# waiwnf/pilotguru

Measured on AMD Instinct MI355X. Metric: frames/sec ORB extract+match, 1080p @ 2000 kp/frame, higher is better.
Workload: dtype u8

## Files before the change

include/pgorb.h:

```cpp
#ifndef PGORB_H
#define PGORB_H
#include <stdint.h>
#ifdef __cplusplus
extern "C" {
#endif

#define PGORB_MAX_LEVELS 16

enum {
    PGORB_OK = 0,
    PGORB_E_ARG = -1,
    PGORB_E_TOOSMALL = -2,
    PGORB_E_CAP = -3,
    PGORB_E_NODEVICE = -4,
    PGORB_E_HIP = -5,
    PGORB_E_LIMIT = -6,
    PGORB_E_OVERFLOW = -7
};

typedef struct pgorb_ctx pgorb_ctx;

typedef struct pgorb_params {
    int32_t nfeatures;
    float   scale_factor;
// ... 421 lines not shown
#define PGORB_OPTION_UNKNOWN (-2147483647 - 1)
int  pgorb_set_option(pgorb_ctx* ctx, const char* key, int value);
int  pgorb_get_option(const pgorb_ctx* ctx, const char* key);
int  pgorb_matcher_is_popcount(const pgorb_ctx* ctx, int cap_per_frame);

int  pgorb_profile_host(pgorb_ctx* ctx, double* us , int reset);

int  pgorb_debug_level_size(const pgorb_ctx* ctx, int level, int* w, int* h);
int  pgorb_debug_level_image(pgorb_ctx* ctx, int frame, int level, uint8_t* out );
int  pgorb_debug_level_candidates(pgorb_ctx* ctx, int frame, int level,
                                  int32_t* x, int32_t* y, int32_t* response, int cap);
int  pgorb_debug_level_keypoints(pgorb_ctx* ctx, int frame, int level);
int  pgorb_debug_sincos_checksum(uint32_t first_bits, uint32_t count, int nblocks, unsigned long long* out);

enum { PGORB_ARENA_STAGE_A = 0, PGORB_ARENA_PINNED = 1, PGORB_ARENA_SCRATCH = 2, PGORB_ARENA_STAGE_OUT = 3, PGORB_ARENA_XDESC = 4,
       PGORB_ARENA_OUT_BLOCK = 5, PGORB_ARENA_VOCAB = 6, PGORB_ARENA_PLAN_PYR = 7, PGORB_ARENA_PLAN_TABLES = 8 };
int  pgorb_debug_arena(const pgorb_ctx* ctx, int which, const void** ptr, int64_t* bytes);
int  pgorb_debug_host_graph(const pgorb_ctx* ctx, int* last_call, int* plan_epoch);

#ifdef __cplusplus
}
#endif
#endif
```

pilotguru_amd/csrc/extract.hip:

```cpp
#include "pgorb_ctx.h"

#include <chrono>

namespace {

std::vector<hipEvent_t*> pipe_pyr_events(pgorb_ctx* c)
{
    std::vector<hipEvent_t*> v{&c->evFork, &c->evPyrDone, &c->evFastDone};
    for (hipEvent_t& e : c->evLevel) v.push_back(&e);
    return v;
}
std::vector<hipEvent_t*> pipe_lev_events(pgorb_ctx* c)
{
    std::vector<hipEvent_t*> v{&c->evDescDone};
    for (hipEvent_t& e : c->evGrpFast) v.push_back(&e);
    for (hipEvent_t& e : c->evGrpQt) v.push_back(&e);
    return v;
}
int make_side_streams(pgorb_ctx* c, hipStream_t* a, bool aHigh, hipStream_t* b, const std::vector<hipEvent_t*>& events)
{
    int lo = 0, hi = 0;
    PG_HIP(c, hipDeviceGetStreamPriorityRange(&lo, &hi));
    PG_HIP(c, hipStreamCreateWithPriority(a, hipStreamNonBlocking, aHigh ? hi : lo));
    PG_HIP(c, hipStreamCreateWithPriority(b, hipStreamNonBlocking, lo));
// ... 378 lines not shown

int pgorb_debug_level_keypoints(pgorb_ctx* c, int frame, int level)
{
    if (!tap_ok(c, level) || frame < 0 || frame >= c->lastFrames) return PGORB_E_ARG;
    PG_HIP(c, hipSetDevice(c->prm.device));
    PG_HIP(c, hipDeviceSynchronize());
    int32_t cnt = 0;
    PG_HIP(c, hipMemcpy(&cnt, c->plan.kpCount + frame * PG_MAXL + level, 4, hipMemcpyDeviceToHost));
    return cnt;
}

int pgorb_debug_arena(const pgorb_ctx* c, int which, const void** ptr, int64_t* bytes)
{
    if (!c || !ptr || !bytes) return PGORB_E_ARG;
    if (which == PGORB_ARENA_PINNED) { *ptr = c->pinned; *bytes = (int64_t)c->pinnedBytes; return 0; }
    const Arena* all[] = {&c->stageA, nullptr, &c->stageSfi, &c->stageOut, &c->xdesc, &c->outBlk, &c->vocab, &c->pyr, &c->tables};
    if (which < 0 || which >= (int)(sizeof(all) / sizeof(all[0]))) return PGORB_E_ARG;
    *ptr = all[which]->p; *bytes = (int64_t)all[which]->bytes;
    return 0;
}

int pgorb_debug_host_graph(const pgorb_ctx* c, int* last_call, int* plan_epoch)
{
    if (!c || !last_call || !plan_epoch) return PGORB_E_ARG;
    *last_call = c->hg.last; *plan_epoch = c->planEpoch;
    return 0;
}

}
```

pilotguru_amd/csrc/pgorb_internal.h:

```cpp
#pragma once
#include <hip/hip_runtime.h>
#include <stdint.h>
#include <string.h>
#include "../../include/pgorb.h"

#define PG_EDGE 16
#define PG_MAXL PGORB_MAX_LEVELS

struct PgQuadTab {
    int32_t  base_dw;
    uint32_t offs;
    int16_t  a0[4], a1[4];
};

struct PgQuadTab2 {
    int32_t  xb;
    uint32_t sel[4];
    uint32_t coef[4];
};

struct PgRowGrp {
    int32_t  sFirst;
    uint32_t yrel4;
    int16_t  ybeta[8];
// ... 79 lines not shown
    uint2*    qtLeaf;
    int32_t   qtSplit;
    int32_t   qtThreads;
    int32_t   qtWide;
    int32_t*  status;
};

#define QT_PYR_CAP 4096
__host__ __device__ __forceinline__ int qt_pyr_off(int nIni, int d) { return nIni * (((1 << (2 * d)) - 1) / 3); }
__host__ __device__ __forceinline__ int qt_pyr_depth(int nIni)
{
    int D = 5;
    while (D > 0 && qt_pyr_off(nIni, D + 1) > QT_PYR_CAP) D--;
    return D;
}
#if defined(__HIP_DEVICE_COMPILE__)
#define PG_FDIV_RN(a, b) __fdiv_rn(a, b)
#define PG_FMUL_RN(a, b) __fmul_rn(a, b)
#else
#define PG_FDIV_RN(a, b) ((a) / (b))
#define PG_FMUL_RN(a, b) ((a) * (b))
#endif
__host__ __device__ inline uint2 qt_tab_entry(bool isY, int c, float hX, int nIni, int regionH, int D, int wCell, int hCell, int nCols)
{
    const uint32_t mW = ((1u << 20) + wCell - 1) / wCell, mH = ((1u << 20) + hCell - 1) / hCell;
    int part, a0, a1;
    if (isY) { part = 0; a0 = 0; a1 = regionH; }
    else {
        int r = nIni >= 1 ? (int)PG_FDIV_RN((float)c, hX) : 0;
        const int top = (nIni > 1 ? nIni : 1) - 1;
// ... 154 lines not shown
```

pilotguru_amd/csrc/plan.hip:

```cpp
#include "pgorb_ctx.h"

static inline int cvRound(double v) { return (int)lrint(v); }
static inline int cvFloor(double v) { int i = (int)v; return i - (v < i); }

int level_geometry(const pgorb_ctx* c, int w, int h, LevelGeom* g)
{
    for (int l = 0; l < c->prm.nlevels; l++) {
        const float scale = c->mvInvScaleFactor[l];
        g[l].w = cvRound((double)((float)w * scale)); g[l].h = cvRound((double)((float)h * scale));
        const float width = (float)(g[l].w - 2 * PG_EDGE), height = (float)(g[l].h - 2 * PG_EDGE);
        const int nCols = (int)(width / 30.f), nRows = (int)(height / 30.f);
        if (nCols < 1 || nRows < 1) return PGORB_E_TOOSMALL;
        g[l].nCols = nCols; g[l].nRows = nRows;
        g[l].wCell = (int)ceilf(width / nCols);
        g[l].hCell = (int)ceilf(height / nRows);
        const int rw = g[l].w - 2 * PG_EDGE, rh = g[l].h - 2 * PG_EDGE;
        g[l].nIni = (int)roundf((float)rw / rh);
        if (g[l].nIni < 1) g[l].nIni = 0;
        g[l].hX = g[l].nIni ? (float)rw / g[l].nIni : 0.f;
    }
    return 0;
}

namespace {
// ... 208 lines not shown
        A.pyrOff[l] = A.pyrFrame;
        A.pyrFrame += (size_t)V.fstride;
        V.nCols = g[l].nCols; V.nRows = g[l].nRows; V.wCell = g[l].wCell; V.hCell = g[l].hCell;
        V.cellBase = A.cells; A.cells += V.nCols * V.nRows;
        V.quota = c->mnFeaturesPerLevel[l];
        V.nIni = g[l].nIni; V.hX = g[l].hX;
        V.selCap = std::max(V.quota + 2, 4 * V.nIni);
        V.nodeCap = (int)align_up(V.selCap + 8, 4);
        V.candCap = ((V.w - 2 * PG_EDGE) / 2 + V.nCols + 1) * ((V.h - 2 * PG_EDGE) / 2 + V.nRows + 1);
        V.candOff = (int64_t)A.candFrame; A.candFrame += align_up(V.candCap, 64);
        V.cellCap = ((V.wCell + 1) / 2) * ((V.hCell + 1) / 2);
        V.cellCandOff = (int64_t)A.cellCandFrame;
        A.cellCandFrame += align_up((size_t)V.cellCap * V.nCols * V.nRows, 64);
        V.selOff = (int64_t)A.selFrame; A.selFrame += V.selCap;
        V.nodeOff = -1;
        const size_t qtAux = std::max((size_t)3072, (size_t)g[0].nCols * g[0].nRows + 1);
        const size_t qtTab = (size_t)2 * ((g[0].w - 2 * PG_EDGE) + (g[0].h - 2 * PG_EDGE));
        if (std::max((size_t)V.nodeCap * 28, qtTab) * sizeof(int) + qtAux * sizeof(int) + 17 * 1024 > 160 * 1024) {
            V.nodeOff = (int64_t)A.nodeFrame;
            A.nodeFrame += align_up((size_t)V.nodeCap * 30, 64);
        }
        V.scale = c->mvScaleFactor[l];
        V.patchSize = (float)(int)(31 * c->mvScaleFactor[l]);
        A.selTotal += V.selCap;
        if ((size_t)(V.nCols * V.nRows + 1) * sizeof(int) > 140 * 1024)
            return fail(c, PGORB_E_LIMIT, "too many cells on one level for the quadtree kernel's LDS budget");
        if (V.w > 4095 + 2 * PG_EDGE || V.h > 4095 + 2 * PG_EDGE)
            return fail(c, PGORB_E_LIMIT, "level larger than 4095 px is not supported");
        if (V.selCap > 65535)
            return fail(c, PGORB_E_LIMIT, "more than 65533 keypoints on one pyramid level are not supported");
    }
    A.selFrame = align_up(A.selFrame, 16);
    P.totalCells = A.cells; P.selTotal = A.selTotal;
    P.cellCandFrame = (int64_t)A.cellCandFrame;
    P.candFrame = (int64_t)A.candFrame; P.selFrame = (int64_t)A.selFrame; P.nodeFrame = (int64_t)A.nodeFrame;
// ... 187 lines not shown
```

pilotguru_amd/csrc/quadtree.hip:

```cpp
#include "pgorb_internal.h"

#define QT_TMAX 1024
#define QT_T ((int)blockDim.x)
#define QT_SH (__builtin_ctz(blockDim.x))
#define QT_W (QT_T >> 6)
#define QT_POS_MASK 0x0FFFFFFFu

#ifndef QT_HU
#define QT_HU 4
#endif
#define QT_SETTLE4(a, b, c, d) asm volatile("" : "+v"(a), "+v"(b), "+v"(c), "+v"(d))

__device__ __forceinline__ int qt_wave_incl_scan(int x)
{
    int v = x;
    v += __builtin_amdgcn_update_dpp(0, v, 0x111, 0xf, 0xf, true);
    v += __builtin_amdgcn_update_dpp(0, v, 0x112, 0xf, 0xf, true);
    v += __builtin_amdgcn_update_dpp(0, v, 0x114, 0xf, 0xf, true);
    v += __builtin_amdgcn_update_dpp(0, v, 0x118, 0xf, 0xf, true);
    v += __builtin_amdgcn_update_dpp(0, v, 0x142, 0xa, 0xf, false);
    v += __builtin_amdgcn_update_dpp(0, v, 0x143, 0xc, 0xf, false);
    return v;
}

__device__ int qt_scan_excl(int* a, int n, int* sh)
{
    const int tid = threadIdx.x, lane = tid & 63, wv = tid >> 6;
    const int per = (n + QT_T - 1) >> QT_SH;
    const int b = tid * per, e = min(b + per, n);
    int sum = 0;
    for (int i = b; i < e; i++) sum += a[i];
    const int incl = qt_wave_incl_scan(sum);
    if (lane == 63) sh[wv] = incl;
    __syncthreads();
    if (wv == 0) {
        const int v = (lane < QT_W) ? sh[lane] : 0;
        const int w = qt_wave_incl_scan(v);
        if (lane < QT_W) sh[lane] = w - v;
        if (lane == QT_W - 1) sh[QT_W] = w;
    }
    __syncthreads();
    int run = sh[wv] + incl - sum;
    for (int i = b; i < e; i++) { const int v = a[i]; a[i] = run; run += v; }
    const int total = sh[QT_W];
    __syncthreads();
    return total;
}

__device__ __forceinline__ void qt_scan3_threads(int& a, int& b, int& c, int* tot, int* sh)
{
    const int tid = threadIdx.x, lane = tid & 63, wv = tid >> 6;
    const int ia = qt_wave_incl_scan(a), ib = qt_wave_incl_scan(b), ic = qt_wave_incl_scan(c);
    if (lane == 63) { sh[wv] = ia; sh[QT_W + wv] = ib; sh[2 * QT_W + wv] = ic; }
    __syncthreads();
    int pa = 0, pb = 0, pc = 0, ta = 0, tb = 0, tc = 0;
    for (int w = 0; w < QT_W; w++) {
        const int va = sh[w], vb = sh[QT_W + w], vc = sh[2 * QT_W + w];
        if (w < wv) { pa += va; pb += vb; pc += vc; }
// ... 4 lines not shown
    __syncthreads();
}

__device__ __forceinline__ void qt_wave_count(int* ctr, int target, bool active)
{
    const unsigned long long todo = __ballot(active);
    if (todo == 0) return;
    const int leader = __ffsll((long long)todo) - 1;
    const int t = __builtin_amdgcn_readlane(target, leader);
    if (__ballot(active && target != t) == 0) {
        if ((int)(threadIdx.x & 63) == leader) atomicAdd(&ctr[t], __popcll(todo));
    } else if (active) {
        atomicAdd(&ctr[target], 1);
    }
}

__device__ __forceinline__ int qt_quadrant(const int4 b, uint32_t cv)
{
    const int midX = b.x + ((b.z - b.x + 1) >> 1);
    const int midY = b.y + ((b.w - b.y + 1) >> 1);
    const int x = cv & 0xFFF, y = (cv >> 12) & 0xFFF;
    return (x < midX) ? ((y < midY) ? 0 : 2) : ((y < midY) ? 1 : 3);
}


__device__ __forceinline__ int qt_leaf(uint32_t cv, float hX, int nIni, int regionH, int D)
{
    const int x = cv & 0xFFF, y = (cv >> 12) & 0xFFF;
    int r = (int)__fdiv_rn((float)x, hX);
    r = min(max(r, 0), nIni - 1);
// ... 9 lines not shown
    return idx;
}

__device__ __forceinline__ int qt_walk(const int* map, int leaf, int nIni, int D)
{
    for (int d = 0; d <= D; d++) {
        const int m = map[qt_pyr_off(nIni, d) + (leaf >> (2 * (D - d)))];
        if (m >= 0) return m;
    }
    return 0;
}

__device__ __forceinline__ int qt_build_keys(const int32_t* __restrict__ cc, const uint32_t* __restrict__ slots, int ncells, int cellCap,
                                             int* cellOff, int* sh, uint2* keys, float hX, int nIni, int regionH, int D)
{
    const int tid = threadIdx.x;
    for (int i = tid; i < ncells; i += QT_T) cellOff[i] = min(cc[i], cellCap);
    __syncthreads();
    const int ncand = qt_scan_excl(cellOff, ncells, sh);
    if (tid == 0) cellOff[ncells] = ncand;
    __syncthreads();
    int steps = 0;
    while ((1 << steps) < ncells) steps++;
    for (int b0 = 0; b0 < ncand; b0 += QT_HU * QT_T) {
        int lo[QT_HU], hi[QT_HU];
#pragma unroll
        for (int u = 0; u < QT_HU; u++) { lo[u] = 0; hi[u] = ncells - 1; }
        for (int st = 0; st < steps; st++) {
#pragma unroll
            for (int u = 0; u < QT_HU; u++) {
                const int mid = (lo[u] + hi[u] + 1) >> 1;
                const bool le = cellOff[mid] <= b0 + u * QT_T + tid;
                lo[u] = le ? mid : lo[u];
                hi[u] = le ? hi[u] : mid - 1;
            }
        }
        uint32_t v[QT_HU];
#pragma unroll
// ... 2 lines not shown
            v[u] = (i < ncand) ? slots[(int64_t)lo[u] * cellCap + (i - cellOff[lo[u]])] : 0u;
        }
        QT_SETTLE4(v[0], v[1], v[2], v[3]);
        if (QT_HU == 8) QT_SETTLE4(v[4 % QT_HU], v[5 % QT_HU], v[6 % QT_HU], v[7 % QT_HU]);
#pragma unroll
        for (int u = 0; u < QT_HU; u++) {
            const int i = b0 + u * QT_T + tid;
            if (i < ncand) keys[i] = make_uint2(v[u], (uint32_t)qt_leaf(v[u], hX, nIni, regionH, D));
        }
    }
    __syncthreads();
    return ncand;
}

template <bool BIG, int WIDE>
__global__ __launch_bounds__((WIDE == 1 || WIDE == 3) ? 512 : QT_TMAX, WIDE == 3 ? 6 : (WIDE ? 4 : 8)) void k_quadtree(const PgPlan P, int level0, int leafOffInts, int split)
{
    __shared__ int sh[3 * (QT_TMAX / 64) + 8];
    __shared__ int pyr[QT_PYR_CAP];
    extern __shared__ __attribute__((aligned(16))) int qt_lds[];
    const int tid = threadIdx.x;
    const int l = level0 + blockIdx.y, frame = blockIdx.x;
    const PgLevel& L = P.lvl[l];
    int* kpc = &P.kpCount[frame * PG_MAXL + l];
    uint2* keys = reinterpret_cast<uint2*>(P.cand) + ((int64_t)frame * P.candFrame + L.candOff);
    if (BIG != (L.nodeOff >= 0)) return;
    const int NC = L.nodeCap;
    int* nodeBase = BIG ? P.nodeScratch + (int64_t)frame * P.nodeFrame + L.nodeOff : qt_lds;
    int4* bndA = reinterpret_cast<int4*>(nodeBase);
    int4* bndB = bndA + NC;
    int* cntA = reinterpret_cast<int*>(bndB + NC);
    int* cntB = cntA + NC;
    int* pidA = cntB + NC;
    int* pidB = pidA + NC;
    int* cnt4 = pidB + NC;
    int* cnt4n = cnt4 + 4 * NC;
    int* newpos4 = cnt4n + 4 * NC;
    int* tailpos = newpos4 + 4 * NC;
    int* rnk = tailpos + NC;
    int* ord = rnk + NC;
    int* cinc = ord + NC;
    int* tmp = newpos4;
    int* ecnt = newpos4 + NC;
    unsigned long long* best = reinterpret_cast<unsigned long long*>(newpos4);
    uint32_t* leafBest = reinterpret_cast<uint32_t*>(qt_lds + leafOffInts);
    int* cellOff = qt_lds + leafOffInts;

    const int N = L.quota;
    const int regionH = L.h - 2 * PG_EDGE;
    const int nIni = L.nIni;
    const float hX = L.hX;
    const int D = qt_pyr_depth(nIni);
    const int pyrTotal = qt_pyr_off(nIni, D + 1);

    const int wCell = L.wCell, hCell = L.hCell, nCols = L.nCols;
    const uint32_t mW = ((1u << 20) + wCell - 1) / wCell, mH = ((1u << 20) + hCell - 1) / hCell;
    auto order_rank = [&](uint32_t cv) {
        const uint32_t x = (cv & 0xFFF) - 3, y = ((cv >> 12) & 0xFFF) - 3;
        const uint32_t cj = (x * mW) >> 20, ci = (y * mH) >> 20;
        return ((ci * nCols + cj) * hCell + (y - ci * hCell)) * wCell + (x - cj * wCell);
    };
// ... 10 lines not shown
        for (int i = tid; i < pyrTotal; i += QT_T) pyr[i] = 0;
        if (!split) for (int i = tid; i < nleaf; i += QT_T) leafBest[i] = 0u;
        if (tid == 0) sh[QT_W + 2] = 0;
        int mine = 0;
        const int lane = tid & 63;
        if (split) {
            __syncthreads();
            int* hDs = pyr + qt_pyr_off(nIni, D);
            uint2* gl = P.qtLeaf + ((int64_t)frame * P.nlevels + l) * PG_QT_LEAF_CAP;
            for (int i = tid; i < nleaf; i += QT_T) {
                const uint2 e = gl[i];
                hDs[i] = (int)e.x; leafBest[i] = e.y; mine += (int)e.x;
            }
        } else {
        const int regionW = L.w - 2 * PG_EDGE;
        uint2* xTab = reinterpret_cast<uint2*>(qt_lds);
        uint2* yTab = xTab + regionW;
        for (int i = tid; i < regionW + regionH; i += QT_T) {
            const bool isY = i >= regionW;
            const int c = isY ? i - regionW : i;
            (isY ? yTab : xTab)[c] = qt_tab_entry(isY, c, hX, nIni, regionH, D, wCell, hCell, nCols);
        }
        __syncthreads();
        int* hD = pyr + qt_pyr_off(nIni, D);
        const int wv = __builtin_amdgcn_readfirstlane(tid >> 6);
        const int cellCap = L.cellCap;
        struct __attribute__((packed, aligned(4))) U4 { uint32_t e[4]; };
        if (ncells < QT_T) {
            const int sub = lane >> 4, sl = lane & 15;
            const int cpw = (((ncells + QT_W - 1) >> (QT_SH - 6)) + 31) & ~31;
            const int cBeg = wv * cpw, cEnd = min(ncells, cBeg + cpw);
// ... 90 lines not shown
        for (int d = D - 1; d >= 0; d--) {
            const int* src = pyr + qt_pyr_off(nIni, d + 1);
            int* dst = pyr + qt_pyr_off(nIni, d);
            const int cnt = nIni << (2 * d);
            for (int j = tid; j < cnt; j += QT_T) dst[j] = src[4 * j] + src[4 * j + 1] + src[4 * j + 2] + src[4 * j + 3];
            __syncthreads();
        }
    }

    int size;
    {
        if (tid == 0) {
            int pos = 0;
            for (int i = 0; i < nIni; i++) {
                if (pyr[i] > 0) {
                    bndA[pos] = make_int4((int)__fmul_rn(hX, (float)i), 0,
                                          (int)__fmul_rn(hX, (float)(i + 1)), regionH);
                    cntA[pos] = pyr[i];
                    pidA[pos] = i;
                    pos++;
                }
            }
            sh[QT_W + 1] = pos;
        }
        __syncthreads();
        size = sh[QT_W + 1];
        if (D >= 1)
            for (int i = tid; i < 4 * size; i += QT_T) cnt4[i] = pyr[nIni + 4 * pidA[i >> 2] + (i & 3)];
        __syncthreads();
    }

    int sorted_mode = 0, gen = 1;
    bool last = false, pyrMode = true;
    while (!last) {
        if (pyrMode && gen > D) {
            if (!keysBuilt) {
                qt_build_keys(P.cellCount + (int64_t)frame * P.totalCells + L.cellBase, P.cellCand + (int64_t)frame * P.cellCandFrame + L.cellCandOff,
                              L.nCols * L.nRows, L.cellCap, cellOff, sh, keys, hX, nIni, regionH, D);
                keysBuilt = true;
            }
            for (int i = tid; i < pyrTotal; i += QT_T) pyr[i] = -1;
            for (int i = tid; i < 4 * size; i += QT_T) cnt4[i] = 0;
            __syncthreads();
            for (int p = tid; p < size; p += QT_T) {
                const int pid = pidA[p];
                pyr[qt_pyr_off(nIni, pid >> 28) + (pid & QT_POS_MASK)] = p;
            }
            __syncthreads();
            for (int i0 = 0; i0 < ncand; i0 += QT_T) {
                const int i = i0 + tid;
                bool act = i < ncand;
                int tgt = 0;
                if (act) {
                    const uint2 k = keys[i];
                    const int pos = qt_walk(pyr, (int)k.y, nIni, D);
                    uint32_t rec = (uint32_t)pos;
                    act = cntA[pos] > 1;
                    if (act) {
                        const int q = qt_quadrant(bndA[pos], k.x);
                        tgt = pos * 4 + q;
                        rec |= (uint32_t)q << 28;
                    }
                    keys[i].y = rec;
                }
                qt_wave_count(cnt4, tgt, act);
            }
            __syncthreads();
            pyrMode = false;
        }
        const int n = size, prevSize = size;
        const bool fill = pyrMode && gen + 1 <= D;
        const int fillOff = qt_pyr_off(nIni, min(gen + 1, D));
        int jstar = 0;
        if (!sorted_mode) {
// ... 3 lines not shown
            for (int p = pb; p < pe; p++)
                if (cntA[p] > 1) {
                    const int c0 = cnt4[4 * p], c1 = cnt4[4 * p + 1], c2 = cnt4[4 * p + 2], c3 = cnt4[4 * p + 3];
                    se++; sc += (c0 > 0) + (c1 > 0) + (c2 > 0) + (c3 > 0); sx += (c0 > 1) + (c1 > 1) + (c2 > 1) + (c3 > 1);
                }
            int tot[3];
            qt_scan3_threads(se, sc, sx, tot, sh);
            const int m = tot[0], Ctot = tot[1], nToExpand = tot[2];
            size = Ctot + (n - m);
            if (size > NC) { if (tid == 0) atomicExch(P.status, PGORB_E_OVERFLOW); size = min(size, NC); last = true; }
            if (size >= N || size == prevSize) last = true;
            else if (size + 3 * nToExpand > N) sorted_mode = 1;
            int re = se, ce = sc;
            for (int p = pb; p < pe; p++) {
                if (cntA[p] > 1) {
                    const int4 b = bndA[p];
                    const int midX = b.x + ((b.z - b.x + 1) >> 1);
                    const int midY = b.y + ((b.w - b.y + 1) >> 1);
                    const int cq[4] = {cnt4[4 * p], cnt4[4 * p + 1], cnt4[4 * p + 2], cnt4[4 * p + 3]};
                    const int c = (cq[0] > 0) + (cq[1] > 0) + (cq[2] > 0) + (cq[3] > 0);
                    const int cidx = (int)(((uint32_t)pidA[p] & (QT_POS_MASK >> 2)) * 4u);
                    int pos = Ctot - (ce + c);
                    if (pos >= 0 && pos + c <= NC) {
#pragma unroll
                        for (int q = 3; q >= 0; q--) {
                            if (cq[q] <= 0) continue;
                            bndB[pos] = make_int4((q & 1) ? midX : b.x, (q & 2) ? midY : b.y,
                                                  (q & 1) ? b.z : midX, (q & 2) ? b.w : midY);
                            cntB[pos] = cq[q];
                            pidB[pos] = (int)(((uint32_t)gen << 28) | (uint32_t)(cidx + q));
                            if (fill && cq[q] > 1) {
                                const int* h = pyr + fillOff + (cidx + q) * 4;
                                cnt4n[4 * pos] = h[0]; cnt4n[4 * pos + 1] = h[1]; cnt4n[4 * pos + 2] = h[2]; cnt4n[4 * pos + 3] = h[3];
                            }
                            newpos4[4 * p + q] = pos++;
                        }
                    }
                    rnk[p] = 0; re++; ce += c;
                } else {
                    const int pos = min(Ctot + (p - re), NC - 1);
                    bndB[pos] = bndA[p]; cntB[pos] = cntA[p]; pidB[pos] = pidA[p];
                    tailpos[p] = pos; rnk[p] = -1;
                }
            }
        } else {
            for (int p = tid; p < n; p += QT_T) rnk[p] = (cntA[p] > 1) ? 1 : 0;
            __syncthreads();
            const int m = qt_scan_excl(rnk, n, sh);
            if (BIG) {
                for (int p = tid; p < n; p += QT_T) {
                    if (cntA[p] > 1) { tmp[rnk[p]] = p; ecnt[rnk[p]] = cntA[p]; }
                    else rnk[p] = -1;
                }
                __syncthreads();
                for (int i = tid; i < m; i += QT_T) {
                    const int ci = ecnt[i];
                    int rank = 0;
                    for (int j = 0; j < m; j++) {
                        const int cj = ecnt[j];
                        rank += (cj > ci) || (cj == ci && j < i);
                    }
                    ord[rank] = tmp[i];
                    rnk[tmp[i]] = rank;
                }
                __syncthreads();
            } else {
                for (int p = tid; p < n; p += QT_T) {
                    if (cntA[p] > 1) { tmp[rnk[p]] = p; ecnt[rnk[p]] = (int)(((uint32_t)min(cntA[p], 0x1FFFFF) << 11) | (uint32_t)(2047 - rnk[p])); }
                    else rnk[p] = -1;
                }
                __syncthreads();
                const int m4 = m & ~3;
                for (int i = tid; i < m; i += QT_T) {
                    const uint32_t ki = (uint32_t)ecnt[i];
                    int rank = 0;
                    for (int j = 0; j < m4; j += 4) {
                        const uint4 k4 = *reinterpret_cast<const uint4*>(ecnt + j);
                        rank += (k4.x > ki) + (k4.y > ki) + (k4.z > ki) + (k4.w > ki);
                    }
                    for (int j = m4; j < m; j++) rank += (uint32_t)ecnt[j] > ki;
                    ord[rank] = tmp[i];
                    rnk[tmp[i]] = rank;
                }
                __syncthreads();
            }
            for (int r = tid; r < m; r += QT_T) {
                const int p = ord[r];
                cinc[r] = (cnt4[4 * p] > 0) + (cnt4[4 * p + 1] > 0) + (cnt4[4 * p + 2] > 0) + (cnt4[4 * p + 3] > 0);
            }
            __syncthreads();
            qt_scan_excl(cinc, m, sh);
            for (int r = tid; r < m; r += QT_T) {
                const int p = ord[r];
                cinc[r] += (cnt4[4 * p] > 0) + (cnt4[4 * p + 1] > 0) + (cnt4[4 * p + 2] > 0) + (cnt4[4 * p + 3] > 0);
            }
            if (tid == 0) sh[QT_W + 1] = m - 1;
            __syncthreads();
            for (int r = tid; r < m; r += QT_T) {
                const bool now = n + cinc[r] - (r + 1) >= N;
                const bool before = (r > 0) && (n + cinc[r - 1] - r >= N);
                if (now && !before) sh[QT_W + 1] = r;
            }
            __syncthreads();
            jstar = sh[QT_W + 1];
            const int Ctot = (m > 0) ? cinc[jstar] : 0;
            for (int p = tid; p < n; p += QT_T) tailpos[p] = (rnk[p] >= 0 && rnk[p] <= jstar) ? 0 : 1;
            __syncthreads();
            const int U = qt_scan_excl(tailpos, n, sh);
            for (int p = tid; p < n; p += QT_T) {
                const int r = rnk[p];
                if (r >= 0 && r <= jstar) {
                    const int4 b = bndA[p];
                    const int midX = b.x + ((b.z - b.x + 1) >> 1);
                    const int midY = b.y + ((b.w - b.y + 1) >> 1);
                    const int cq[4] = {cnt4[4 * p], cnt4[4 * p + 1], cnt4[4 * p + 2], cnt4[4 * p + 3]};
                    const int cidx = (int)(((uint32_t)pidA[p] & (QT_POS_MASK >> 2)) * 4u);
                    int pos = Ctot - cinc[r];
#pragma unroll
                    for (int q = 3; q >= 0; q--) {
                        if (cq[q] <= 0) continue;
                        bndB[pos] = make_int4((q & 1) ? midX : b.x, (q & 2) ? midY : b.y,
                                              (q & 1) ? b.z : midX, (q & 2) ? b.w : midY);
                        cntB[pos] = cq[q];
                        pidB[pos] = (int)(((uint32_t)gen << 28) | (uint32_t)(cidx + q));
                        if (fill && cq[q] > 1) {
                            const int* h = pyr + fillOff + (cidx + q) * 4;
                            cnt4n[4 * pos] = h[0]; cnt4n[4 * pos + 1] = h[1]; cnt4n[4 * pos + 2] = h[2]; cnt4n[4 * pos + 3] = h[3];
                        }
                        newpos4[4 * p + q] = pos++;
                    }
                } else {
                    const int pos = Ctot + tailpos[p];
                    bndB[pos] = bndA[p]; cntB[pos] = cntA[p]; pidB[pos] = pidA[p];
                    tailpos[p] = pos;
                    if (fill && cntA[p] > 1) {
                        cnt4n[4 * pos] = cnt4[4 * p]; cnt4n[4 * pos + 1] = cnt4[4 * p + 1];
                        cnt4n[4 * pos + 2] = cnt4[4 * p + 2]; cnt4n[4 * pos + 3] = cnt4[4 * p + 3];
                    }
                }
            }
            size = Ctot + U;
            if (size > NC) { if (tid == 0) atomicExch(P.status, PGORB_E_OVERFLOW); size = NC; last = true; }
            if (size >= N || size == prevSize) last = true;
        }
        if (!pyrMode) {
            for (int i = tid; i < 4 * size; i += QT_T) cnt4n[i] = 0;
            __syncthreads();
            for (int b0 = 0; b0 < ncand; b0 += 4 * QT_T) {
                uint2 kk[4];
#pragma unroll
                for (int u = 0; u < 4; u++) { const int i = b0 + tid + u * QT_T; kk[u] = (i < ncand) ? keys[i] : make_uint2(0u, 0u); }
        QT_SETTLE4(kk[0].x, kk[1].x, kk[2].x, kk[3].x); QT_SETTLE4(kk[0].y, kk[1].y, kk[2].y, kk[3].y);
                int tgt[4];
                bool act[4];
#pragma unroll
                for (int u = 0; u < 4; u++) {
                    const int i = b0 + tid + u * QT_T;
                    act[u] = i < ncand;
                    tgt[u] = 0;
                    if (act[u]) {
                        const uint2 k = kk[u];
                        const int pos = k.y & QT_POS_MASK, q = k.y >> 28;
                        const int r = rnk[pos];
                        const int np = (r >= 0 && r <= jstar) ? newpos4[4 * pos + q] : tailpos[pos];
                        uint32_t rec = (uint32_t)np;
                        act[u] = !last && cntB[np] > 1;
                        if (act[u]) {
                            const int q2 = qt_quadrant(bndB[np], k.x);
                            tgt[u] = np * 4 + q2;
                            rec |= (uint32_t)q2 << 28;
                        }
                        if (last) atomicMax(&reinterpret_cast<unsigned long long*>(cnt4n)[np], bid(k.x));
                        else keys[i].y = rec;
                    }
                }
#pragma unroll
                for (int u = 0; u < 4; u++) qt_wave_count(cnt4n, tgt[u], act[u]);
            }
        }
        __syncthreads();
        { int4* t4 = bndA; bndA = bndB; bndB = t4; int* t1 = cntA; cntA = cntB; cntB = t1;
          t1 = cnt4; cnt4 = cnt4n; cnt4n = t1; t1 = pidA; pidA = pidB; pidB = t1; }
        gen++;
    }

    if (pyrMode) {
        for (int p = tid; p < size; p += QT_T) best[p] = 0ull;
        int* leafPos = pyr + qt_pyr_off(nIni, D);
        for (int i = tid; i < pyrTotal; i += QT_T) pyr[i] = -1;
        __syncthreads();
        for (int p = tid; p < size; p += QT_T) {
            const int pid = pidA[p];
            pyr[qt_pyr_off(nIni, pid >> 28) + (pid & QT_POS_MASK)] = p;
        }
        __syncthreads();
        const int nleaf = nIni << (2 * D);
// ... 152 lines not shown
    }
    __syncthreads();
    uint2* gl = P.qtLeaf + ((int64_t)frame * P.nlevels + l) * PG_QT_LEAF_CAP;
    const uint32_t cmask = (1u << D) - 1;
    for (int i = tid; i < nh; i += QTP_T) {
        const uint32_t rl = (uint32_t)i / (uint32_t)ncol, col = (uint32_t)i - rl * (uint32_t)ncol, row = (uint32_t)r0 + rl;
        const uint32_t leaf = ((col >> D) << (2 * D)) + qt_spread_bits(col & cmask) + 2u * qt_spread_bits(row);
        gl[leaf] = make_uint2((uint32_t)hC[i], hB[i]);
    }
}

void pg_launch_quadtree(const PgPlan& P, int nframes, hipStream_t s) { pg_launch_quadtree_levels(P, nframes, 0, P.nlevels, s); }

void pg_launch_quadtree_levels(const PgPlan& P, int nframes, int levelBeg, int levelEnd, hipStream_t s)
{
    int nodes[2] = {0, 0}, aux[2] = {0, 0};
    bool any[2] = {false, false};
    for (int l = levelBeg; l < levelEnd; l++) {
        const int big = P.lvl[l].nodeOff >= 0 ? 1 : 0;
        const int cells = P.lvl[l].nCols * P.lvl[l].nRows + 1;
        const int nIni = max(P.lvl[l].nIni, 1);
        const int leaves = nIni << (2 * qt_pyr_depth(nIni));
        any[big] = true;
        aux[big] = max(aux[big], max(cells, leaves));
        nodes[big] = max(nodes[big], 2 * ((P.lvl[l].w - 2 * PG_EDGE) + (P.lvl[l].h - 2 * PG_EDGE)));
        if (!big) nodes[0] = max(nodes[0], P.lvl[l].nodeCap * 28);
    }
    static size_t configuredDev[64] = {0};
    int dev = 0;
    (void)hipGetDevice(&dev);
    size_t& configured = configuredDev[dev & 63];
    const int cells0 = P.lvl[levelBeg].nCols * P.lvl[levelBeg].nRows;
    const bool split = P.qtSplit == 1 || (P.qtSplit == 2 && cells0 >= 1500 && nframes <= 16 + (cells0 - 2304) * 12 / 6912);
    if (split) {
        int groups = 0;
        size_t lds = 0;
        for (int l = levelBeg; l < levelEnd; l++) {
            const PgLevel& V = P.lvl[l];
            const int D = qt_pyr_depth(V.nIni), ncells = V.nCols * V.nRows;
            groups += qt_pass_groups(ncells, D);
            lds = std::max(lds, (size_t)((V.w - 2 * PG_EDGE) + (V.h - 2 * PG_EDGE)) * 8 + (size_t)qt_pass_rows_per_group(ncells, D) * (std::max(V.nIni, 0) << D) * 8 + 2 * 64 * 4);
        }
        static size_t passConfigured[64] = {0};
        int dev0 = 0;
        (void)hipGetDevice(&dev0);
        if (lds > 48 * 1024 && lds > passConfigured[dev0 & 63]) {
            (void)hipFuncSetAttribute(reinterpret_cast<const void*>(k_qt_leaves), hipFuncAttributeMaxDynamicSharedMemorySize, (int)lds);
            passConfigured[dev0 & 63] = lds;
        }
        if (groups > 0)
            hipLaunchKernelGGL(k_qt_leaves, dim3(groups, nframes), dim3(QTP_T), lds, s, P, levelBeg, levelEnd - levelBeg);
    }
    for (int big = 0; big < 2; big++) {
        if (!any[big]) continue;
        const size_t lds = (size_t)(nodes[big] + aux[big]) * sizeof(int);
        const size_t ldsAll = lds + sizeof(int) * (QT_PYR_CAP + 3 * (QT_TMAX / 64) + 8);
        int threads = QT_TMAX;
        if (ldsAll <= 80 * 1024 && (cells0 < 1024 || (int64_t)nframes * (levelEnd - levelBeg) > 256)) threads = 512;
        if (P.qtThreads == 256 || P.qtThreads == 512 || P.qtThreads == 1024) threads = P.qtThreads;
        dim3 grid(nframes, levelEnd - levelBeg), block(threads);
        const int64_t problems = (int64_t)nframes * (levelEnd - levelBeg);
        int wide = 0;
        if (P.qtWide && threads == 512 && ldsAll > 54 * 1024) wide = 1;
        if (P.qtWide && threads == 512 && ldsAll > 40 * 1024 && ldsAll <= 54 * 1024) wide = 3;
        if (P.qtWide && threads == QT_TMAX && (ldsAll > 80 * 1024 || problems <= 256)) wide = 2;
        if (lds > configured) {
#define PG_QT_ATTR(B, W) (void)hipFuncSetAttribute(reinterpret_cast<const void*>(k_quadtree<B, W>), hipFuncAttributeMaxDynamicSharedMemorySize, (int)lds)
            PG_QT_ATTR(true, 0); PG_QT_ATTR(true, 1); PG_QT_ATTR(true, 2); PG_QT_ATTR(true, 3); PG_QT_ATTR(false, 0); PG_QT_ATTR(false, 1); PG_QT_ATTR(false, 2); PG_QT_ATTR(false, 3);
#undef PG_QT_ATTR
            configured = lds;
        }
#define PG_QT_LAUNCH(B, W) hipLaunchKernelGGL((k_quadtree<B, W>), grid, block, lds, s, P, levelBeg, nodes[big], split ? 1 : 0)
        if (big) { if (wide == 1) PG_QT_LAUNCH(true, 1); else if (wide == 2) PG_QT_LAUNCH(true, 2); else if (wide == 3) PG_QT_LAUNCH(true, 3); else PG_QT_LAUNCH(true, 0); }
        else { if (wide == 1) PG_QT_LAUNCH(false, 1); else if (wide == 2) PG_QT_LAUNCH(false, 2); else if (wide == 3) PG_QT_LAUNCH(false, 3); else PG_QT_LAUNCH(false, 0); }
#undef PG_QT_LAUNCH
    }
}
```

pilotguru_amd/orb.py:

```python
import ctypes as C
import weakref

import numpy as np

from . import _lib

KEYPOINT_DTYPE = np.dtype([("x", "<f4"), ("y", "<f4"), ("size", "<f4"), ("angle", "<f4"),
                           ("response", "<f4"), ("octave", "<i4"), ("class_id", "<i4")])
assert KEYPOINT_DTYPE.itemsize == 28


def _p(a):
    return C.c_void_p(a.ctypes.data)


def _arr(x, dtype, n, name, width=None):
    a = np.ascontiguousarray(x, dtype)
    if a.shape != ((n,) if width is None else (n, width)):
        raise ValueError("%s: shape %s, expected %s" % (name, a.shape, (n,) if width is None else (n, width)))
    return a


def _frame(F, name):
    return (_arr(F.mvKeysUndistorted, KEYPOINT_DTYPE, F.N, name + " keypoints"),
# ... 217 lines not shown
        w, h = self.debug_level_size(level)
        out = np.zeros((h, w), np.uint8)
        self._check(self._L.pgorb_debug_level_image(self._h, frame, level, _p(out)))
        return out

    def debug_level_candidates(self, frame, level):
        w, h = self.debug_level_size(level)
        cap = w * h // 2 + 64
        x, y, r = (np.zeros(cap, np.int32) for _ in range(3))
        n = self._check(self._L.pgorb_debug_level_candidates(self._h, frame, level, _p(x), _p(y), _p(r), cap))
        return x[:n].copy(), y[:n].copy(), r[:n].copy()

    def debug_level_keypoints(self, frame, level):
        return self._check(self._L.pgorb_debug_level_keypoints(self._h, frame, level))

    ARENAS = ("stageA", "pinned", "stageSfi", "stageOut", "xdesc", "outBlk", "vocab", "plan_pyr", "plan_tables")

    def debug_arena(self, name):
        ptr, n = C.c_void_p(), C.c_int64()
        self._check(self._L.pgorb_debug_arena(self._h, self.ARENAS.index(name), C.byref(ptr), C.byref(n)))
        return ptr.value or 0, n.value

    def debug_host_graph(self):
        last, epoch = C.c_int32(), C.c_int32()
        self._check(self._L.pgorb_debug_host_graph(self._h, C.byref(last), C.byref(epoch)))
        return last.value, epoch.value

    def hamming_matrix(self, a, b):
        a = np.ascontiguousarray(a, np.uint8).reshape(-1, 32)
        b = np.ascontiguousarray(b, np.uint8).reshape(-1, 32)
        out = np.zeros((len(a), len(b)), np.uint16)
# ... 608 lines not shown
```

Before: 97900.

## Compact quadtree LDS layout with 16-bit bounds and indices, dynamic pyramid sizing

Shrinks the quadtree kernel's shared-memory footprint. Node bounds are packed into uint2 with 16-bit coordinates, per-node rank and position arrays become uint16, and the separate ord array is removed by computing child counts during ranking. The fixed static pyramid array is moved into dynamic LDS sized per launch, and the node-spill threshold and thread and wide-mode heuristics are recomputed. This allows more levels to keep nodes in LDS and raises occupancy, at the cost of 16-bit overflow limits and added pack/unpack arithmetic.

```diff
diff --git a/include/pgorb.h b/include/pgorb.h
--- a/include/pgorb.h
+++ b/include/pgorb.h
@@ -459,7 +459,8 @@
 int  pgorb_debug_sincos_checksum(uint32_t first_bits, uint32_t count, int nblocks, unsigned long long* out);
 
 enum { PGORB_ARENA_STAGE_A = 0, PGORB_ARENA_PINNED = 1, PGORB_ARENA_SCRATCH = 2, PGORB_ARENA_STAGE_OUT = 3, PGORB_ARENA_XDESC = 4,
-       PGORB_ARENA_OUT_BLOCK = 5, PGORB_ARENA_VOCAB = 6, PGORB_ARENA_PLAN_PYR = 7, PGORB_ARENA_PLAN_TABLES = 8 };
+       PGORB_ARENA_OUT_BLOCK = 5, PGORB_ARENA_VOCAB = 6, PGORB_ARENA_PLAN_PYR = 7, PGORB_ARENA_PLAN_TABLES = 8,
+       PGORB_ARENA_PLAN_NODES = 9 };
 int  pgorb_debug_arena(const pgorb_ctx* ctx, int which, const void** ptr, int64_t* bytes);
 int  pgorb_debug_host_graph(const pgorb_ctx* ctx, int* last_call, int* plan_epoch);
 
diff --git a/pilotguru_amd/csrc/extract.hip b/pilotguru_amd/csrc/extract.hip
--- a/pilotguru_amd/csrc/extract.hip
+++ b/pilotguru_amd/csrc/extract.hip
@@ -416,7 +416,7 @@
 {
     if (!c || !ptr || !bytes) return PGORB_E_ARG;
     if (which == PGORB_ARENA_PINNED) { *ptr = c->pinned; *bytes = (int64_t)c->pinnedBytes; return 0; }
-    const Arena* all[] = {&c->stageA, nullptr, &c->stageSfi, &c->stageOut, &c->xdesc, &c->outBlk, &c->vocab, &c->pyr, &c->tables};
+    const Arena* all[] = {&c->stageA, nullptr, &c->stageSfi, &c->stageOut, &c->xdesc, &c->outBlk, &c->vocab, &c->pyr, &c->tables, &c->nodes};
     if (which < 0 || which >= (int)(sizeof(all) / sizeof(all[0]))) return PGORB_E_ARG;
     *ptr = all[which]->p; *bytes = (int64_t)all[which]->bytes;
     return 0;
diff --git a/pilotguru_amd/csrc/pgorb_internal.h b/pilotguru_amd/csrc/pgorb_internal.h
--- a/pilotguru_amd/csrc/pgorb_internal.h
+++ b/pilotguru_amd/csrc/pgorb_internal.h
@@ -117,6 +117,17 @@
     while (D > 0 && qt_pyr_off(nIni, D + 1) > QT_PYR_CAP) D--;
     return D;
 }
+__host__ __device__ __forceinline__ int qt_node_ints(int nodeCap) { return 19 * nodeCap + nodeCap / 2 + 2; }
+__host__ __device__ __forceinline__ int qt_node_area_ints(int nodeCap, int cells, int w, int h, bool hbmNodes)
+{
+    const int tab = 2 * ((w - 2 * PG_EDGE) + (h - 2 * PG_EDGE));
+    int a = tab > cells + 1 ? tab : cells + 1;
+    if (!hbmNodes) {
+        a = a > qt_node_ints(nodeCap) ? a : qt_node_ints(nodeCap);
+        a = a > 8 * nodeCap + cells + 1 ? a : 8 * nodeCap + cells + 1;
+    }
+    return a;
+}
 #if defined(__HIP_DEVICE_COMPILE__)
 #define PG_FDIV_RN(a, b) __fdiv_rn(a, b)
 #define PG_FMUL_RN(a, b) __fmul_rn(a, b)
diff --git a/pilotguru_amd/csrc/plan.hip b/pilotguru_amd/csrc/plan.hip
--- a/pilotguru_amd/csrc/plan.hip
+++ b/pilotguru_amd/csrc/plan.hip
@@ -246,11 +246,10 @@
         A.cellCandFrame += align_up((size_t)V.cellCap * V.nCols * V.nRows, 64);
         V.selOff = (int64_t)A.selFrame; A.selFrame += V.selCap;
         V.nodeOff = -1;
-        const size_t qtAux = std::max((size_t)3072, (size_t)g[0].nCols * g[0].nRows + 1);
-        const size_t qtTab = (size_t)2 * ((g[0].w - 2 * PG_EDGE) + (g[0].h - 2 * PG_EDGE));
-        if (std::max((size_t)V.nodeCap * 28, qtTab) * sizeof(int) + qtAux * sizeof(int) + 17 * 1024 > 160 * 1024) {
+        const size_t qtArea = (size_t)qt_node_area_ints(V.nodeCap, g[0].nCols * g[0].nRows, g[0].w, g[0].h, false);
+        if ((qtArea + 3072 + QT_PYR_CAP) * sizeof(int) + 1024 > 160 * 1024) {
             V.nodeOff = (int64_t)A.nodeFrame;
-            A.nodeFrame += align_up((size_t)V.nodeCap * 30, 64);
+            A.nodeFrame += align_up((size_t)qt_node_ints(V.nodeCap), 64);
         }
         V.scale = c->mvScaleFactor[l];
         V.patchSize = (float)(int)(31 * c->mvScaleFactor[l]);
diff --git a/pilotguru_amd/csrc/quadtree.hip b/pilotguru_amd/csrc/quadtree.hip
--- a/pilotguru_amd/csrc/quadtree.hip
+++ b/pilotguru_amd/csrc/quadtree.hip
@@ -5,6 +5,7 @@
 #define QT_SH (__builtin_ctz(blockDim.x))
 #define QT_W (QT_T >> 6)
 #define QT_POS_MASK 0x0FFFFFFFu
+#define QT_NONE 0xFFFFu
 
 #ifndef QT_HU
 #define QT_HU 4
@@ -23,12 +24,14 @@
     return v;
 }
 
-__device__ int qt_scan_excl(int* a, int n, int* sh)
+template <class T>
+__device__ int qt_scan_excl(T* a, int n, int* sh)
 {
     const int tid = threadIdx.x, lane = tid & 63, wv = tid >> 6;
     const int per = (n + QT_T - 1) >> QT_SH;
     const int b = tid * per, e = min(b + per, n);
     int sum = 0;
+#pragma nounroll
     for (int i = b; i < e; i++) sum += a[i];
     const int incl = qt_wave_incl_scan(sum);
     if (lane == 63) sh[wv] = incl;
@@ -41,7 +44,8 @@
     }
     __syncthreads();
     int run = sh[wv] + incl - sum;
-    for (int i = b; i < e; i++) { const int v = a[i]; a[i] = run; run += v; }
+#pragma nounroll
+    for (int i = b; i < e; i++) { const int v = a[i]; a[i] = sizeof(T) == 2 ? (T)min(run, 0xFFFF) : (T)run; run += v; }
     const int total = sh[QT_W];
     __syncthreads();
     return total;
@@ -76,6 +80,9 @@
         atomicAdd(&ctr[target], 1);
     }
 }
+
+__device__ __forceinline__ uint2 qt_pack_bounds(int x0, int y0, int x1, int y1) { return make_uint2((uint32_t)x0 | ((uint32_t)x1 << 16), (uint32_t)y0 | ((uint32_t)y1 << 16)); }
+__device__ __forceinline__ int4 qt_unpack_bounds(const uint2 b) { return make_int4((int)(b.x & 0xFFFFu), (int)(b.y & 0xFFFFu), (int)(b.x >> 16), (int)(b.y >> 16)); }
 
 __device__ __forceinline__ int qt_quadrant(const int4 b, uint32_t cv)
 {
@@ -115,7 +122,9 @@
 __device__ __forceinline__ int qt_build_keys(const int32_t* __restrict__ cc, const uint32_t* __restrict__ slots, int ncells, int cellCap,
                                              int* cellOff, int* sh, uint2* keys, float hX, int nIni, int regionH, int D)
 {
-    const int tid = threadIdx.x;
+    int tid = threadIdx.x;
+    asm volatile("" : "+v"(tid));
+#pragma nounroll
     for (int i = tid; i < ncells; i += QT_T) cellOff[i] = min(cc[i], cellCap);
     __syncthreads();
     const int ncand = qt_scan_excl(cellOff, ncells, sh);
@@ -123,6 +132,7 @@
     __syncthreads();
     int steps = 0;
     while ((1 << steps) < ncells) steps++;
+#pragma nounroll
     for (int b0 = 0; b0 < ncand; b0 += QT_HU * QT_T) {
         int lo[QT_HU], hi[QT_HU];
 #pragma unroll
@@ -155,11 +165,12 @@
 }
 
 template <bool BIG, int WIDE>
-__global__ __launch_bounds__((WIDE == 1 || WIDE == 3) ? 512 : QT_TMAX, WIDE == 3 ? 6 : (WIDE ? 4 : 8)) void k_quadtree(const PgPlan P, int level0, int leafOffInts, int split)
+__global__ __launch_bounds__((WIDE == 1 || WIDE == 3) ? 512 : QT_TMAX, WIDE == 3 ? 6 : (WIDE ? 4 : 8)) void k_quadtree(const PgPlan P, int level0, int areaOffInts, int leafOffInts, int split)
 {
     __shared__ int sh[3 * (QT_TMAX / 64) + 8];
-    __shared__ int pyr[QT_PYR_CAP];
     extern __shared__ __attribute__((aligned(16))) int qt_lds[];
+    int* pyr = qt_lds;
+    int* area = qt_lds + areaOffInts;
     const int tid = threadIdx.x;
     const int l = level0 + blockIdx.y, frame = blockIdx.x;
     const PgLevel& L = P.lvl[l];
@@ -167,25 +178,24 @@
     uint2* keys = reinterpret_cast<uint2*>(P.cand) + ((int64_t)frame * P.candFrame + L.candOff);
     if (BIG != (L.nodeOff >= 0)) return;
     const int NC = L.nodeCap;
-    int* nodeBase = BIG ? P.nodeScratch + (int64_t)frame * P.nodeFrame + L.nodeOff : qt_lds;
-    int4* bndA = reinterpret_cast<int4*>(nodeBase);
-    int4* bndB = bndA + NC;
+    int* nodeBase = BIG ? P.nodeScratch + (int64_t)frame * P.nodeFrame + L.nodeOff : area;
+    uint2* bndA = reinterpret_cast<uint2*>(nodeBase);
+    uint2* bndB = bndA + NC;
     int* cntA = reinterpret_cast<int*>(bndB + NC);
     int* cntB = cntA + NC;
     int* pidA = cntB + NC;
     int* pidB = pidA + NC;
     int* cnt4 = pidB + NC;
     int* cnt4n = cnt4 + 4 * NC;
-    int* newpos4 = cnt4n + 4 * NC;
-    int* tailpos = newpos4 + 4 * NC;
-    int* rnk = tailpos + NC;
-    int* ord = rnk + NC;
-    int* cinc = ord + NC;
-    int* tmp = newpos4;
-    int* ecnt = newpos4 + NC;
+    uint16_t* newpos4 = reinterpret_cast<uint16_t*>(nodeBase + 16 * NC);
+    uint16_t* tailpos = newpos4 + 4 * NC;
+    uint16_t* rnk = tailpos + NC;
+    uint16_t* cinc = rnk + NC;
+    int* tmp = reinterpret_cast<int*>(newpos4);
+    int* ecnt = tmp + NC;
     unsigned long long* best = reinterpret_cast<unsigned long long*>(newpos4);
     uint32_t* leafBest = reinterpret_cast<uint32_t*>(qt_lds + leafOffInts);
-    int* cellOff = qt_lds + leafOffInts;
+    int* cellOff = BIG ? area : area + 8 * NC;
 
     const int N = L.quota;
     const int regionH = L.h - 2 * PG_EDGE;
@@ -226,7 +236,7 @@
             }
         } else {
         const int regionW = L.w - 2 * PG_EDGE;
-        uint2* xTab = reinterpret_cast<uint2*>(qt_lds);
+        uint2* xTab = reinterpret_cast<uint2*>(area);
         uint2* yTab = xTab + regionW;
         for (int i = tid; i < regionW + regionH; i += QT_T) {
             const bool isY = i >= regionW;
@@ -347,8 +357,8 @@
             int pos = 0;
             for (int i = 0; i < nIni; i++) {
                 if (pyr[i] > 0) {
-                    bndA[pos] = make_int4((int)__fmul_rn(hX, (float)i), 0,
-                                          (int)__fmul_rn(hX, (float)(i + 1)), regionH);
+                    bndA[pos] = qt_pack_bounds((int)__fmul_rn(hX, (float)i), 0,
+                                               (int)__fmul_rn(hX, (float)(i + 1)), regionH);
                     cntA[pos] = pyr[i];
                     pidA[pos] = i;
                     pos++;
@@ -372,16 +382,21 @@
                               L.nCols * L.nRows, L.cellCap, cellOff, sh, keys, hX, nIni, regionH, D);
                 keysBuilt = true;
             }
-            for (int i = tid; i < pyrTotal; i += QT_T) pyr[i] = -1;
-            for (int i = tid; i < 4 * size; i += QT_T) cnt4[i] = 0;
-            __syncthreads();
-            for (int p = tid; p < size; p += QT_T) {
+            int tidL = tid;
+            asm volatile("" : "+v"(tidL));
+#pragma nounroll
+            for (int i = tidL; i < pyrTotal; i += QT_T) pyr[i] = -1;
+#pragma nounroll
+            for (int i = tidL; i < 4 * size; i += QT_T) cnt4[i] = 0;
+            __syncthreads();
+            for (int p = tidL; p < size; p += QT_T) {
                 const int pid = pidA[p];
                 pyr[qt_pyr_off(nIni, pid >> 28) + (pid & QT_POS_MASK)] = p;
             }
             __syncthreads();
+#pragma nounroll
             for (int i0 = 0; i0 < ncand; i0 += QT_T) {
-                const int i = i0 + tid;
+                const int i = i0 + tidL;
                 bool act = i < ncand;
                 int tgt = 0;
                 if (act) {
@@ -390,7 +405,7 @@
                     uint32_t rec = (uint32_t)pos;
                     act = cntA[pos] > 1;
                     if (act) {
-                        const int q = qt_quadrant(bndA[pos], k.x);
+                        const int q = qt_quadrant(qt_unpack_bounds(bndA[pos]), k.x);
                         tgt = pos * 4 + q;
                         rec |= (uint32_t)q << 28;
                     }
@@ -424,7 +439,7 @@
             int re = se, ce = sc;
             for (int p = pb; p < pe; p++) {
                 if (cntA[p] > 1) {
-                    const int4 b = bndA[p];
+                    const int4 b = qt_unpack_bounds(bndA[p]);
                     const int midX = b.x + ((b.z - b.x + 1) >> 1);
                     const int midY = b.y + ((b.w - b.y + 1) >> 1);
                     const int cq[4] = {cnt4[4 * p], cnt4[4 * p + 1], cnt4[4 * p + 2], cnt4[4 * p + 3]};
@@ -435,22 +450,22 @@
 #pragma unroll
                         for (int q = 3; q >= 0; q--) {
                             if (cq[q] <= 0) continue;
-                            bndB[pos] = make_int4((q & 1) ? midX : b.x, (q & 2) ? midY : b.y,
-                                                  (q & 1) ? b.z : midX, (q & 2) ? b.w : midY);
+                            bndB[pos] = qt_pack_bounds((q & 1) ? midX : b.x, (q & 2) ? midY : b.y,
+                                                       (q & 1) ? b.z : midX, (q & 2) ? b.w : midY);
                             cntB[pos] = cq[q];
                             pidB[pos] = (int)(((uint32_t)gen << 28) | (uint32_t)(cidx + q));
                             if (fill && cq[q] > 1) {
                                 const int* h = pyr + fillOff + (cidx + q) * 4;
                                 cnt4n[4 * pos] = h[0]; cnt4n[4 * pos + 1] = h[1]; cnt4n[4 * pos + 2] = h[2]; cnt4n[4 * pos + 3] = h[3];
                             }
-                            newpos4[4 * p + q] = pos++;
+                            newpos4[4 * p + q] = (uint16_t)pos++;
                         }
                     }
                     rnk[p] = 0; re++; ce += c;
                 } else {
                     const int pos = min(Ctot + (p - re), NC - 1);
                     bndB[pos] = bndA[p]; cntB[pos] = cntA[p]; pidB[pos] = pidA[p];
-                    tailpos[p] = pos; rnk[p] = -1;
+                    tailpos[p] = (uint16_t)pos; rnk[p] = QT_NONE;
                 }
             }
         } else {
@@ -460,7 +475,7 @@
             if (BIG) {
                 for (int p = tid; p < n; p += QT_T) {
                     if (cntA[p] > 1) { tmp[rnk[p]] = p; ecnt[rnk[p]] = cntA[p]; }
-                    else rnk[p] = -1;
+                    else rnk[p] = QT_NONE;
                 }
                 __syncthreads();
                 for (int i = tid; i < m; i += QT_T) {
@@ -470,14 +485,15 @@
                         const int cj = ecnt[j];
                         rank += (cj > ci) || (cj == ci && j < i);
                     }
-                    ord[rank] = tmp[i];
-                    rnk[tmp[i]] = rank;
+                    const int p = tmp[i];
+                    rnk[p] = (uint16_t)rank;
+                    cinc[rank] = (uint16_t)((cnt4[4 * p] > 0) + (cnt4[4 * p + 1] > 0) + (cnt4[4 * p + 2] > 0) + (cnt4[4 * p + 3] > 0));
                 }
                 __syncthreads();
             } else {
                 for (int p = tid; p < n; p += QT_T) {
                     if (cntA[p] > 1) { tmp[rnk[p]] = p; ecnt[rnk[p]] = (int)(((uint32_t)min(cntA[p], 0x1FFFFF) << 11) | (uint32_t)(2047 - rnk[p])); }
-                    else rnk[p] = -1;
+                    else rnk[p] = QT_NONE;
                 }
                 __syncthreads();
                 const int m4 = m & ~3;
@@ -489,60 +505,52 @@
                         rank += (k4.x > ki) + (k4.y > ki) + (k4.z > ki) + (k4.w > ki);
                     }
                     for (int j = m4; j < m; j++) rank += (uint32_t)ecnt[j] > ki;
-                    ord[rank] = tmp[i];
-                    rnk[tmp[i]] = rank;
+                    const int p = tmp[i];
+                    rnk[p] = (uint16_t)rank;
+                    cinc[rank] = (uint16_t)((cnt4[4 * p] > 0) + (cnt4[4 * p + 1] > 0) + (cnt4[4 * p + 2] > 0) + (cnt4[4 * p + 3] > 0));
                 }
                 __syncthreads();
             }
+            const int ctotAll = qt_scan_excl(cinc, m, sh);
+            if (tid == 0) { cinc[m] = (uint16_t)min(ctotAll, 0xFFFF); sh[QT_W + 1] = m - 1; }
+            __syncthreads();
             for (int r = tid; r < m; r += QT_T) {
-                const int p = ord[r];
-                cinc[r] = (cnt4[4 * p] > 0) + (cnt4[4 * p + 1] > 0) + (cnt4[4 * p + 2] > 0) + (cnt4[4 * p + 3] > 0);
-            }
-            __syncthreads();
-            qt_scan_excl(cinc, m, sh);
-            for (int r = tid; r < m; r += QT_T) {
-                const int p = ord[r];
-                cinc[r] += (cnt4[4 * p] > 0) + (cnt4[4 * p + 1] > 0) + (cnt4[4 * p + 2] > 0) + (cnt4[4 * p + 3] > 0);
-            }
-            if (tid == 0) sh[QT_W + 1] = m - 1;
-            __syncthreads();
-            for (int r = tid; r < m; r += QT_T) {
-                const bool now = n + cinc[r] - (r + 1) >= N;
-                const bool before = (r > 0) && (n + cinc[r - 1] - r >= N);
+                const bool now = n + (int)cinc[r + 1] - (r + 1) >= N;
+                const bool before = (r > 0) && (n + (int)cinc[r] - r >= N);
                 if (now && !before) sh[QT_W + 1] = r;
             }
             __syncthreads();
             jstar = sh[QT_W + 1];
-            const int Ctot = (m > 0) ? cinc[jstar] : 0;
-            for (int p = tid; p < n; p += QT_T) tailpos[p] = (rnk[p] >= 0 && rnk[p] <= jstar) ? 0 : 1;
+            const int Ctot = (m > 0) ? (int)cinc[jstar + 1] : 0;
+            for (int p = tid; p < n; p += QT_T) tailpos[p] = (rnk[p] != QT_NONE && (int)rnk[p] <= jstar) ? 0 : 1;
             __syncthreads();
             const int U = qt_scan_excl(tailpos, n, sh);
             for (int p = tid; p < n; p += QT_T) {
                 const int r = rnk[p];
-                if (r >= 0 && r <= jstar) {
-                    const int4 b = bndA[p];
+                if (r != (int)QT_NONE && r <= jstar) {
+                    const int4 b = qt_unpack_bounds(bndA[p]);
                     const int midX = b.x + ((b.z - b.x + 1) >> 1);
                     const int midY = b.y + ((b.w - b.y + 1) >> 1);
                     const int cq[4] = {cnt4[4 * p], cnt4[4 * p + 1], cnt4[4 * p + 2], cnt4[4 * p + 3]};
                     const int cidx = (int)(((uint32_t)pidA[p] & (QT_POS_MASK >> 2)) * 4u);
-                    int pos = Ctot - cinc[r];
+                    int pos = Ctot - (int)cinc[r + 1];
 #pragma unroll
                     for (int q = 3; q >= 0; q--) {
                         if (cq[q] <= 0) continue;
-                        bndB[pos] = make_int4((q & 1) ? midX : b.x, (q & 2) ? midY : b.y,
-                                              (q & 1) ? b.z : midX, (q & 2) ? b.w : midY);
+                        bndB[pos] = qt_pack_bounds((q & 1) ? midX : b.x, (q & 2) ? midY : b.y,
+                                                   (q & 1) ? b.z : midX, (q & 2) ? b.w : midY);
                         cntB[pos] = cq[q];
                         pidB[pos] = (int)(((uint32_t)gen << 28) | (uint32_t)(cidx + q));
                         if (fill && cq[q] > 1) {
                             const int* h = pyr + fillOff + (cidx + q) * 4;
                             cnt4n[4 * pos] = h[0]; cnt4n[4 * pos + 1] = h[1]; cnt4n[4 * pos + 2] = h[2]; cnt4n[4 * pos + 3] = h[3];
                         }
-                        newpos4[4 * p + q] = pos++;
+                        newpos4[4 * p + q] = (uint16_t)pos++;
                     }
                 } else {
                     const int pos = Ctot + tailpos[p];
                     bndB[pos] = bndA[p]; cntB[pos] = cntA[p]; pidB[pos] = pidA[p];
-                    tailpos[p] = pos;
+                    tailpos[p] = (uint16_t)pos;
                     if (fill && cntA[p] > 1) {
                         cnt4n[4 * pos] = cnt4[4 * p]; cnt4n[4 * pos + 1] = cnt4[4 * p + 1];
                         cnt4n[4 * pos + 2] = cnt4[4 * p + 2]; cnt4n[4 * pos + 3] = cnt4[4 * p + 3];
@@ -556,6 +564,7 @@
         if (!pyrMode) {
             for (int i = tid; i < 4 * size; i += QT_T) cnt4n[i] = 0;
             __syncthreads();
+#pragma nounroll
             for (int b0 = 0; b0 < ncand; b0 += 4 * QT_T) {
                 uint2 kk[4];
 #pragma unroll
@@ -572,11 +581,11 @@
                         const uint2 k = kk[u];
                         const int pos = k.y & QT_POS_MASK, q = k.y >> 28;
                         const int r = rnk[pos];
-                        const int np = (r >= 0 && r <= jstar) ? newpos4[4 * pos + q] : tailpos[pos];
+                        const int np = (r != (int)QT_NONE && r <= jstar) ? (int)newpos4[4 * pos + q] : (int)tailpos[pos];
                         uint32_t rec = (uint32_t)np;
                         act[u] = !last && cntB[np] > 1;
                         if (act[u]) {
-                            const int q2 = qt_quadrant(bndB[np], k.x);
+                            const int q2 = qt_quadrant(qt_unpack_bounds(bndB[np]), k.x);
                             tgt[u] = np * 4 + q2;
                             rec |= (uint32_t)q2 << 28;
                         }
@@ -589,7 +598,7 @@
             }
         }
         __syncthreads();
-        { int4* t4 = bndA; bndA = bndB; bndB = t4; int* t1 = cntA; cntA = cntB; cntB = t1;
+        { uint2* t4 = bndA; bndA = bndB; bndB = t4; int* t1 = cntA; cntA = cntB; cntB = t1;
           t1 = cnt4; cnt4 = cnt4n; cnt4n = t1; t1 = pidA; pidA = pidB; pidB = t1; }
         gen++;
     }
@@ -772,7 +781,7 @@
 
 void pg_launch_quadtree_levels(const PgPlan& P, int nframes, int levelBeg, int levelEnd, hipStream_t s)
 {
-    int nodes[2] = {0, 0}, aux[2] = {0, 0};
+    int nodes[2] = {0, 0}, aux[2] = {0, 0}, pyrInts[2] = {0, 0};
     bool any[2] = {false, false};
     for (int l = levelBeg; l < levelEnd; l++) {
         const int big = P.lvl[l].nodeOff >= 0 ? 1 : 0;
@@ -780,10 +789,11 @@
         const int nIni = max(P.lvl[l].nIni, 1);
         const int leaves = nIni << (2 * qt_pyr_depth(nIni));
         any[big] = true;
-        aux[big] = max(aux[big], max(cells, leaves));
-        nodes[big] = max(nodes[big], 2 * ((P.lvl[l].w - 2 * PG_EDGE) + (P.lvl[l].h - 2 * PG_EDGE)));
-        if (!big) nodes[0] = max(nodes[0], P.lvl[l].nodeCap * 28);
-    }
+        aux[big] = max(aux[big], leaves);
+        pyrInts[big] = max(pyrInts[big], qt_pyr_off(nIni, qt_pyr_depth(nIni) + 1));
+        nodes[big] = max(nodes[big], qt_node_area_ints(P.lvl[l].nodeCap, cells - 1, P.lvl[l].w, P.lvl[l].h, big != 0));
+    }
+    for (int big = 0; big < 2; big++) { nodes[big] = (nodes[big] + 3) & ~3; pyrInts[big] = (pyrInts[big] + 3) & ~3; }
     static size_t configuredDev[64] = {0};
     int dev = 0;
     (void)hipGetDevice(&dev);
@@ -811,16 +821,18 @@
     }
     for (int big = 0; big < 2; big++) {
         if (!any[big]) continue;
-        const size_t lds = (size_t)(nodes[big] + aux[big]) * sizeof(int);
-        const size_t ldsAll = lds + sizeof(int) * (QT_PYR_CAP + 3 * (QT_TMAX / 64) + 8);
+        const size_t lds = (size_t)(nodes[big] + aux[big] + pyrInts[big]) * sizeof(int);
+        const size_t ldsAll = lds + sizeof(int) * (3 * (QT_TMAX / 64) + 8);
         int threads = QT_TMAX;
         if (ldsAll <= 80 * 1024 && (cells0 < 1024 || (int64_t)nframes * (levelEnd - levelBeg) > 256)) threads = 512;
+        if (threads == 512 && ldsAll <= 32 * 1024 && (int64_t)nframes * (levelEnd - levelBeg) > 1024) threads = 256;
         if (P.qtThreads == 256 || P.qtThreads == 512 || P.qtThreads == 1024) threads = P.qtThreads;
         dim3 grid(nframes, levelEnd - levelBeg), block(threads);
         const int64_t problems = (int64_t)nframes * (levelEnd - levelBeg);
         int wide = 0;
-        if (P.qtWide && threads == 512 && ldsAll > 54 * 1024) wide = 1;
-        if (P.qtWide && threads == 512 && ldsAll > 40 * 1024 && ldsAll <= 54 * 1024) wide = 3;
+        const size_t third = 160 * 1024 / 3;
+        if (P.qtWide && threads == 512 && ldsAll > third) wide = 1;
+        if (P.qtWide && threads == 512 && ldsAll > 40 * 1024 && ldsAll <= third) wide = 3;
         if (P.qtWide && threads == QT_TMAX && (ldsAll > 80 * 1024 || problems <= 256)) wide = 2;
         if (lds > configured) {
 #define PG_QT_ATTR(B, W) (void)hipFuncSetAttribute(reinterpret_cast<const void*>(k_quadtree<B, W>), hipFuncAttributeMaxDynamicSharedMemorySize, (int)lds)
@@ -828,7 +840,7 @@
 #undef PG_QT_ATTR
             configured = lds;
         }
-#define PG_QT_LAUNCH(B, W) hipLaunchKernelGGL((k_quadtree<B, W>), grid, block, lds, s, P, levelBeg, nodes[big], split ? 1 : 0)
+#define PG_QT_LAUNCH(B, W) hipLaunchKernelGGL((k_quadtree<B, W>), grid, block, lds, s, P, levelBeg, pyrInts[big], pyrInts[big] + nodes[big], split ? 1 : 0)
         if (big) { if (wide == 1) PG_QT_LAUNCH(true, 1); else if (wide == 2) PG_QT_LAUNCH(true, 2); else if (wide == 3) PG_QT_LAUNCH(true, 3); else PG_QT_LAUNCH(true, 0); }
         else { if (wide == 1) PG_QT_LAUNCH(false, 1); else if (wide == 2) PG_QT_LAUNCH(false, 2); else if (wide == 3) PG_QT_LAUNCH(false, 3); else PG_QT_LAUNCH(false, 0); }
 #undef PG_QT_LAUNCH
diff --git a/pilotguru_amd/orb.py b/pilotguru_amd/orb.py
--- a/pilotguru_amd/orb.py
+++ b/pilotguru_amd/orb.py
@@ -255,7 +255,7 @@
     def debug_level_keypoints(self, frame, level):
         return self._check(self._L.pgorb_debug_level_keypoints(self._h, frame, level))
 
-    ARENAS = ("stageA", "pinned", "stageSfi", "stageOut", "xdesc", "outBlk", "vocab", "plan_pyr", "plan_tables")
+    ARENAS = ("stageA", "pinned", "stageSfi", "stageOut", "xdesc", "outBlk", "vocab", "plan_pyr", "plan_tables", "plan_nodes")
 
     def debug_arena(self, name):
         ptr, n = C.c_void_p(), C.c_int64()
```

New measurement: 97820. No clear change (-0.1%).
